# Walter0807/MotionBERT

Hardware: AMD Instinct MI355X
Metric: clips/sec [B,243,17,3] DSTformer fwd+bwd (higher is better)
Workload: dtype bf16; 1 GPU; MotionBERT full DSTformer (dim_feat 512, depth 5, 8 heads, mlp_ratio 2) train step: fwd + bwd + AdamW, 64 clips/GPU x T=243 x J=17, random-init weights, pose loss (mpjpe + 0.5 n_mpjpe + 20 velocity, fused kernel), one-launch flat AdamW; global_batch=64, frames=243, parallelism=dp1

## Files before the change

motionbert_amd/csrc/attention.hip:

```cpp
#include "mbx_common.h"

template <bool SHARED> struct AttnBlock { static constexpr int THREADS = SHARED ? 512 : 256, WAVES = THREADS / 64; };
constexpr int MBX_ATTN_KV_THREADS = 256;
template <bool SHARED> struct AttnBlockKV { static constexpr int THREADS = SHARED ? MBX_ATTN_KV_THREADS : 256, WAVES = THREADS / 64; };

template <typename T> struct AT;
template <> struct AT<bf16_t> { static constexpr int EPC = 8, RB = 8, SZ = 2; };
template <> struct AT<float>  { static constexpr int EPC = 4, RB = 4, SZ = 4; };

template <typename T, int HD> struct BReg;
template <int HD> struct BReg<bf16_t, HD> {
    uint4 v[HD / 16];
    __device__ __forceinline__ void load(const bf16_t* row, int g, bool valid) {
#pragma unroll
        for (int s = 0; s < HD / 16; ++s)
            v[s] = valid ? *reinterpret_cast<const uint4*>(row + 16 * s + 8 * g) : make_uint4(0u, 0u, 0u, 0u);
    }
    static __device__ __forceinline__ float dot(const BReg& a, const BReg& b) {
        float acc = 0.f;
        const uint32_t* x = reinterpret_cast<const uint32_t*>(a.v);
        const uint32_t* y = reinterpret_cast<const uint32_t*>(b.v);
#pragma unroll
        for (int i = 0; i < HD / 4; ++i) {
            acc = fmaf(__uint_as_float(x[i] << 16), __uint_as_float(y[i] << 16), acc);
// ... 499 lines not shown
                tk[c] = *reinterpret_cast<const uint4*>(r3 + C);
                tv[c] = *reinterpret_cast<const uint4*>(r3 + 2 * C);
                td[c] = *reinterpret_cast<const uint4*>(dobase + (size_t)row * ostride + ch * 8);
            }
        }
        if (stats && lane < 3 * HD / 4) {
            const int j = lane / (HD / 4), d = (lane % (HD / 4)) * 4;
            const float4 r = *reinterpret_cast<const float4*>(st_rsum + j * C + P.h * HD + d);
            const float4 b = *reinterpret_cast<const float4*>(st_bias + j * C + P.h * HD + d);
            vec_reg = make_uint4(pack_bf2(r.x, r.y), pack_bf2(r.z, r.w), pack_bf2(-b.x, -b.y), pack_bf2(-b.z, -b.w));
        }
#pragma unroll
        for (int c = 0; c < NPT; ++c) {
            const int idx = lane + c * 64, off = (idx / CHB) * RSTR + (idx % CHB) * 16;
            *reinterpret_cast<uint4*>(qt + off) = tq[c];
            *reinterpret_cast<uint4*>(kt + off) = tk[c];
            *reinterpret_cast<uint4*>(vt + off) = tv[c];
            *reinterpret_cast<uint4*>(dot_ + off) = td[c];
        }
        if (lane < KP) lse_s[lane] = l;
    } else {
        fill_two<T, HD, HD / AT<T>::EPC / 2>(qt, qbase, rstride, kt, qbase + C, rstride, RSTR, P.L, KP, lane, 64);
        fill_two<T, HD, HD / AT<T>::EPC / 2>(vt, qbase + 2 * C, rstride, dot_, dobase, ostride, RSTR, P.L, KP, lane, 64);
        if (stats && lane < 3 * HD / 4) {
            const int j = lane / (HD / 4), d = (lane % (HD / 4)) * 4;
            const float4 r = *reinterpret_cast<const float4*>(st_rsum + j * C + P.h * HD + d);
            const float4 b = *reinterpret_cast<const float4*>(st_bias + j * C + P.h * HD + d);
            vec_reg = make_uint4(pack_bf2(r.x, r.y), pack_bf2(r.z, r.w), pack_bf2(-b.x, -b.y), pack_bf2(-b.z, -b.w));
        }
        if (lane < KP) lse_s[lane] = lane < P.L ? lse[(P.tok0 + (size_t)lane * P.tstep) * H + P.h] : 0.f;
    }
    __syncthreads();
    const bool rvalid = pvalid && i < P.L;
    const size_t tok = P.tok0 + (size_t)min(i, P.L - 1) * P.tstep;

    f32x16_t dq[HD / 32];
    {
        BReg<T, HD> qreg, doreg;
        qreg.load(reinterpret_cast<const T*>(qt + (size_t)i * RSTR), g, true);
        doreg.load(reinterpret_cast<const T*>(dot_ + (size_t)i * RSTR), g, true);
        const float lq = lse_s[i];
        f32x16_t sf, dp;
#pragma unroll
        for (int r = 0; r < 16; ++r) { sf[r] = 0.f; dp[r] = 0.f; }
#pragma unroll
        for (int df = 0; df < HD / 32; ++df)
#pragma unroll
            for (int r = 0; r < 16; ++r) dq[df][r] = 0.f;
        MmaRows<T, HD>::run(kt, RSTR, 0, qreg, lane, sf);
        MmaRows<T, HD>::run(vt, RSTR, 0, doreg, lane, dp);
        float dl = 0.f;
#pragma unroll
        for (int r = 0; r < 16; ++r) {
            const int key = (r & 3) + 8 * (r >> 2) + 4 * g;
            const float pr = (rvalid && key < P.L) ? __expf(sf[r] * scale - lq) : 0.f;
            const float dpr = DROP ? dp[r] * drop_mul(dr, P.dbase, min(i, P.L - 1), min(key, P.L - 1), P.L) : dp[r];
            sf[r] = pr;
            dp[r] = dpr;
            dl = fmaf(pr, dpr, dl);
        }
        const float delta = wave_halves<WaveAdd>(dl);
        if (g == 0) del_s[i] = delta;
#pragma unroll
        for (int r = 0; r < 16; ++r) sf[r] = sf[r] * (dp[r] - delta) * scale;
#pragma unroll
        for (int df = 0; df < HD / 32; ++df) MmaCols<T>::run(kt, RSTR, df * 32, 0, sf, lane, dq[df]);
    }
    {
        BReg<T, HD> kreg, vreg;
        kreg.load(reinterpret_cast<const T*>(kt + (size_t)i * RSTR), g, true);
        vreg.load(reinterpret_cast<const T*>(vt + (size_t)i * RSTR), g, true);
        if (!stats) store_rowfrag<T, HD>(reinterpret_cast<T*>(kt + (size_t)i * RSTR), dq, 1.0f, g);
        f32x16_t sf, dp, dk[HD / 32], dv[HD / 32];
#pragma unroll
        for (int r = 0; r < 16; ++r) { sf[r] = 0.f; dp[r] = 0.f; }
#pragma unroll
        for (int df = 0; df < HD / 32; ++df)
#pragma unroll
            for (int r = 0; r < 16; ++r) { dk[df][r] = 0.f; dv[df][r] = 0.f; }
        MmaRows<T, HD>::run(qt, RSTR, 0, kreg, lane, sf);
        MmaRows<T, HD>::run(dot_, RSTR, 0, vreg, lane, dp);
#pragma unroll
        for (int qd = 0; qd < 4; ++qd) {
            const int q0 = 8 * qd + 4 * g;
            const float4 l4 = *reinterpret_cast<const float4*>(lse_s + q0);
            const float4 d4 = *reinterpret_cast<const float4*>(del_s + q0);
            const float la[4] = {l4.x, l4.y, l4.z, l4.w}, da[4] = {d4.x, d4.y, d4.z, d4.w};
#pragma unroll
            for (int e = 0; e < 4; ++e) {
                const int r = 4 * qd + e;
                const float pr = (rvalid && q0 + e < P.L) ? __expf(sf[r] * scale - la[e]) : 0.f;
                const float km = DROP ? drop_mul(dr, P.dbase, min(q0 + e, P.L - 1), min(i, P.L - 1), P.L) : 1.f;
                dp[r] = pr * (dp[r] * km - da[e]) * scale;
                sf[r] = pr * km;
            }
        }
#pragma unroll
        for (int df = 0; df < HD / 32; ++df) {
            MmaCols<T>::run(dot_, RSTR, df * 32, 0, sf, lane, dv[df]);
            MmaCols<T>::run(qt, RSTR, df * 32, 0, dp, lane, dk[df]);
        }
        if constexpr (sizeof(T) == 2) {
            if (stats) {
                if (lane < 3 * HD / 4) vec[lane] = vec_reg;
                float a1 = 0.f, a2 = 0.f, b1 = 0.f, b2 = 0.f;
                store_rowfrag_dot<HD>(reinterpret_cast<bf16_t*>(qt + (size_t)i * RSTR), dq, g, vec, a1, a2);
                store_rowfrag_dot<HD>(reinterpret_cast<bf16_t*>(kt + (size_t)i * RSTR), dk, g, vec + HD / 4, b1, b2);
                store_rowfrag_dot<HD>(reinterpret_cast<bf16_t*>(vt + (size_t)i * RSTR), dv, g, vec + 2 * (HD / 4), b1, b2);
                a1 = wave_halves<WaveAdd>(a1); a2 = wave_halves<WaveAdd>(a2);
                b1 = wave_halves<WaveAdd>(b1); b2 = wave_halves<WaveAdd>(b2);
                if (rvalid && g == 0) {
                    const size_t Mtot = (size_t)(nprob / H) * P.L;
                    *reinterpret_cast<float2*>(st_part + ((size_t)(2 * P.h) * Mtot + tok) * 2) = make_float2(a1, a2);
                    *reinterpret_cast<float2*>(st_part + ((size_t)(2 * P.h + 1) * Mtot + tok) * 2) = make_float2(b1, b2);
                }
            }
        }
        if (!stats) {
            store_rowfrag<T, HD>(reinterpret_cast<T*>(vt + (size_t)i * RSTR), dk, 1.0f, g);
            store_rowfrag<T, HD>(reinterpret_cast<T*>(qt + (size_t)i * RSTR), dv, 1.0f, g);
        }
    }
    if (pvalid) {
        constexpr int CH = HD * (int)sizeof(T) / 16;
        T* ob = dqkv + P.tok0 * C3 + (size_t)P.h * HD;
        const char* sa = stats ? qt : kt;
        const char* sb = stats ? kt : vt;
        const char* sc = stats ? vt : qt;
        for (int idx = lane; idx < P.L * CH; idx += 64) {
            const int r = idx / CH, ch = idx % CH, off = r * RSTR + ch * 16;
            const uint4 a = *reinterpret_cast<const uint4*>(sa + off);
            const uint4 b = *reinterpret_cast<const uint4*>(sb + off);
            const uint4 c = *reinterpret_cast<const uint4*>(sc + off);
            if (sizeof(T) == 4 && dq_lo) {
                const size_t eo = P.tok0 * C3 + (size_t)P.h * HD + (size_t)r * rstride + ch * 4;
                bf16_t* const hi = reinterpret_cast<bf16_t*>(dqkv);
                const float va[4] = {__uint_as_float(a.x), __uint_as_float(a.y), __uint_as_float(a.z), __uint_as_float(a.w)};
                const float vb[4] = {__uint_as_float(b.x), __uint_as_float(b.y), __uint_as_float(b.z), __uint_as_float(b.w)};
                const float vc[4] = {__uint_as_float(c.x), __uint_as_float(c.y), __uint_as_float(c.z), __uint_as_float(c.w)};
                store4_planes(hi + eo, dq_lo + eo, va);
                store4_planes(hi + eo + C, dq_lo + eo + C, vb);
                store4_planes(hi + eo + 2 * C, dq_lo + eo + 2 * C, vc);
                continue;
            }
            T* dst = ob + (size_t)r * rstride + ch * (16 / (int)sizeof(T));
            *reinterpret_cast<uint4*>(dst) = a;
            *reinterpret_cast<uint4*>(dst + C) = b;
            *reinterpret_cast<uint4*>(dst + 2 * C) = c;
        }
    }
}

__device__ __forceinline__ bf16_t* qt_row(char* tile, int row, int stride) { return reinterpret_cast<bf16_t*>(tile + (size_t)row * stride); }
template <int HD>
__device__ __forceinline__ void mma_rows_ldsb(const char* tile, int stride, int row0, const char* brow, int lane, f32x16_t& acc) {
    const char* p = tile + (size_t)(row0 + (lane & 31)) * stride + (lane >> 5) * 16;
#pragma unroll
    for (int s = 0; s < HD / 16; ++s) {
        const bf16x8_t a = *reinterpret_cast<const bf16x8_t*>(p + s * 32);
        const bf16x8_t b = *reinterpret_cast<const bf16x8_t*>(brow + s * 32);
        acc = __builtin_amdgcn_mfma_f32_32x32x16_bf16(a, b, acc, 0, 0, 0);
    }
}

struct Raw4b {
    static __device__ __forceinline__ void unpack(const uint2& r, float (&v)[4]) {
        v[0] = __uint_as_float(r.x << 16); v[1] = __uint_as_float(r.x & 0xffff0000u);
        v[2] = __uint_as_float(r.y << 16); v[3] = __uint_as_float(r.y & 0xffff0000u);
    }
};
#ifndef MBX_ATTN_DBG
#define MBX_ATTN_DBG 0
#endif
#ifdef MBX_ATTN_TRACE
__device__ long long* g_attn_trace;
#define AT_TS(slot_) do { if (threadIdx.x == 0) ats[slot_] = (long long)wall_clock64(); __builtin_amdgcn_sched_barrier(0); } while (0)
#else
#define AT_TS(slot_) do { } while (0)
#endif
template <int HD, bool STATS>
__global__ __launch_bounds__(1024, 1) void attn_bwd_fused_kernel(const bf16_t* __restrict__ qkv, const bf16_t* __restrict__ o,
                                                                 const bf16_t* __restrict__ d_o, const float* __restrict__ lse,
                                                                 bf16_t* __restrict__ dqkv, int Tn, int J, int H, float scale,
                                                                 int mode, int nprob, int KP, const float* __restrict__ st_bias,
                                                                 const float* __restrict__ st_rsum, float* __restrict__ st_part) {
    typedef bf16_t T;
    constexpr int RSTR = rm_stride<T>(HD), CH = HD / 8;
    extern __shared__ __attribute__((aligned(16))) char smem[];
#ifdef MBX_ATTN_TRACE
    long long ats[8] = {0, 0, 0, 0, 0, 0, 0, 0};
#endif
    AT_TS(0);
    const int tid = threadIdx.x, lane = tid & 63, wave = __builtin_amdgcn_readfirstlane(tid >> 6), g = lane >> 5;
    const int C = H * HD, C3 = 3 * C;
    const Prob P = decode_prob((int)blockIdx.x, mode, Tn, J, H);
    const int TB = KP * RSTR;
    char* qt = smem;
    char* kt = qt + TB;
    char* vt = kt + TB;
    char* dot_ = vt + TB;
    float* lse_s = reinterpret_cast<float*>(dot_ + TB);
    float* del_s = lse_s + KP;
    uint4* vec = reinterpret_cast<uint4*>(del_s + KP);
    const size_t rstride = (size_t)P.tstep * C3, ostride = (size_t)P.tstep * C;
    const T* qbase = qkv + P.tok0 * C3 + (size_t)P.h * HD;
    const T* dobase = d_o + P.tok0 * C + (size_t)P.h * HD;
    const T* obase = o + P.tok0 * C + (size_t)P.h * HD;
    if (STATS) fill_stat_vec<HD>(vec, st_rsum, st_bias, C, P.h, tid, 1024);

    for (int i0 = tid; i0 < KP * CH; i0 += 2048) {
        uint4 v[2][4], vo[2];
        float sl[2] = {0.f, 0.f};
#pragma unroll
        for (int u = 0; u < 2; ++u) {
            const int idx = i0 + u * 1024, row = idx / CH, ch = idx % CH;
#pragma unroll
            for (int t = 0; t < 4; ++t) v[u][t] = make_uint4(0u, 0u, 0u, 0u);
            vo[u] = make_uint4(0u, 0u, 0u, 0u);
            if (idx < KP * CH && row < P.L && !(MBX_ATTN_DBG & 4)) {
                const T* r3 = qbase + (size_t)row * rstride + ch * 8;
                v[u][0] = *reinterpret_cast<const uint4*>(r3);
                v[u][1] = *reinterpret_cast<const uint4*>(r3 + C);
                v[u][2] = *reinterpret_cast<const uint4*>(r3 + 2 * C);
                v[u][3] = *reinterpret_cast<const uint4*>(dobase + (size_t)row * ostride + ch * 8);
                vo[u] = *reinterpret_cast<const uint4*>(obase + (size_t)row * ostride + ch * 8);
                if (ch == 0) sl[u] = lse[(P.tok0 + (size_t)row * P.tstep) * H + P.h];
            }
        }
#pragma unroll
        for (int u = 0; u < 2; ++u) {
            const int idx = i0 + u * 1024, row = idx / CH, ch = idx % CH;
            if (idx < KP * CH) {
                const int off = row * RSTR + ch * 16;
                *reinterpret_cast<uint4*>(qt + off) = v[u][0];
                *reinterpret_cast<uint4*>(kt + off) = v[u][1];
                *reinterpret_cast<uint4*>(vt + off) = v[u][2];
                *reinterpret_cast<uint4*>(dot_ + off) = v[u][3];
            }
        }
        AT_TS(1);
#pragma unroll
        for (int u = 0; u < 2; ++u) {
            const int idx = i0 + u * 1024, row = idx / CH, ch = idx % CH;
            float x[4], y[4], dl = 0.f;
            Raw4b::unpack(make_uint2(v[u][3].x, v[u][3].y), x); Raw4b::unpack(make_uint2(vo[u].x, vo[u].y), y);
            dl = fmaf(x[0], y[0], fmaf(x[1], y[1], fmaf(x[2], y[2], fmaf(x[3], y[3], dl))));
            Raw4b::unpack(make_uint2(v[u][3].z, v[u][3].w), x); Raw4b::unpack(make_uint2(vo[u].z, vo[u].w), y);
            dl = fmaf(x[0], y[0], fmaf(x[1], y[1], fmaf(x[2], y[2], fmaf(x[3], y[3], dl))));
            dl += dpp_mov<0xB1>(dl, dl);
            dl += dpp_mov<0x4E>(dl, dl);
            if (CH == 8) dl += dpp_mov<0x141>(dl, dl);
            if (ch == 0 && idx < KP * CH) {
                lse_s[row] = sl[u] * 1.44269504088896341f;
                del_s[row] = dl;
            }
        }
    }
    __syncthreads();
    AT_TS(2);

    const int nfr = (P.L + 31) / 32;
    const float c2 = scale * 1.44269504088896341f;
    f32x16_t acc[2 * (HD / 32)];
#pragma unroll
    for (int a = 0; a < 2 * (HD / 32); ++a)
#pragma unroll
        for (int r = 0; r < 16; ++r) acc[a][r] = 0.f;
    const bool qrole = wave >= 8;
    const int blk = wave & 7, row = blk * 32 + (lane & 31);
    if (blk < nfr && !(MBX_ATTN_DBG & 1)) {
        if (qrole) {
            BReg<T, HD> qreg, doreg;
            qreg.load(reinterpret_cast<const T*>(qt + (size_t)row * RSTR), g, true);
            doreg.load(reinterpret_cast<const T*>(dot_ + (size_t)row * RSTR), g, true);
            const float delta = del_s[row], lq2 = lse_s[row];
            for (int f = 0; f < nfr; ++f) {
                f32x16_t s, dp;
#pragma unroll
                for (int r = 0; r < 16; ++r) { s[r] = 0.f; dp[r] = 0.f; }
                MmaRows<T, HD>::run(kt, RSTR, 32 * f, qreg, lane, s);
                MmaRows<T, HD>::run(vt, RSTR, 32 * f, doreg, lane, dp);
#pragma unroll
                for (int r = 0; r < 16; ++r) {
                    const float p = __builtin_amdgcn_exp2f(fmaf(s[r], c2, -lq2));
                    s[r] = p * (dp[r] - delta);
                }
#pragma unroll
                for (int df = 0; df < HD / 32; ++df) MmaCols<T>::run(kt, RSTR, df * 32, f, s, lane, acc[df]);
            }
        } else {
            int boff = row * RSTR + g * 16;
            for (int f = 0; f < nfr; ++f) {
                asm volatile("" : "+v"(boff));
                f32x16_t s, dp;
#pragma unroll
                for (int r = 0; r < 16; ++r) { s[r] = 0.f; dp[r] = 0.f; }
                mma_rows_ldsb<HD>(qt, RSTR, 32 * f, kt + boff, lane, s);
                mma_rows_ldsb<HD>(dot_, RSTR, 32 * f, vt + boff, lane, dp);
#pragma unroll
                for (int qd = 0; qd < 4; ++qd) {
                    const int q0 = 32 * f + 8 * qd + 4 * g;
                    const float4 l4 = *reinterpret_cast<const float4*>(lse_s + q0);
                    const float4 d4 = *reinterpret_cast<const float4*>(del_s + q0);
                    const float la[4] = {l4.x, l4.y, l4.z, l4.w}, da[4] = {d4.x, d4.y, d4.z, d4.w};
#pragma unroll
                    for (int e = 0; e < 4; ++e) {
                        const int r = 4 * qd + e;
                        const float p = __builtin_amdgcn_exp2f(fmaf(s[r], c2, -la[e]));
                        dp[r] = p * (dp[r] - da[e]);
                        s[r] = p;
                    }
                }
#pragma unroll
                for (int df = 0; df < HD / 32; ++df) {
                    MmaCols<T>::run(dot_, RSTR, df * 32, f, s, lane, acc[HD / 32 + df]);
                    MmaCols<T>::run(qt, RSTR, df * 32, f, dp, lane, acc[df]);
                }
            }
        }
#pragma unroll
        for (int a = 0; a < HD / 32; ++a)
#pragma unroll
            for (int r = 0; r < 16; ++r) acc[a][r] *= scale;
    }
    AT_TS(3);
#ifdef MBX_ATTN_TRACE
    if (g_attn_trace != nullptr && (threadIdx.x & 63) == 0) g_attn_trace[(size_t)gridDim.x * 9 + (size_t)blockIdx.x * 16 + (threadIdx.x >> 6)] = (long long)wall_clock64();
#endif
    __syncthreads();
    AT_TS(4);
    int tid2 = threadIdx.x;
    asm volatile("" : "+v"(tid2));
    const int g2 = (tid2 >> 5) & 1, row2 = blk * 32 + (tid2 & 31);
    const bool qrole2 = wave >= 8;
    if (blk < nfr) {
        if (STATS) {
            float p1 = 0.f, p2 = 0.f;
            if (qrole2) {
                store_rowfrag_dot<HD>(qt_row(qt, row2, RSTR), reinterpret_cast<const f32x16_t (&)[HD / 32]>(acc[0]), g2, vec, p1, p2);
            } else {
                store_rowfrag_dot<HD>(qt_row(kt, row2, RSTR), reinterpret_cast<const f32x16_t (&)[HD / 32]>(acc[0]), g2, vec + HD / 4, p1, p2);
                store_rowfrag_dot<HD>(qt_row(vt, row2, RSTR), reinterpret_cast<const f32x16_t (&)[HD / 32]>(acc[HD / 32]), g2, vec + 2 * (HD / 4), p1, p2);
            }
            p1 = wave_halves<WaveAdd>(p1);
            p2 = wave_halves<WaveAdd>(p2);
            if (g2 == 0 && row2 < P.L) {
                const size_t Mtot = (size_t)(nprob / H) * P.L;
                *reinterpret_cast<float2*>(st_part + ((size_t)(2 * P.h + (qrole2 ? 0 : 1)) * Mtot + P.tok0 + (size_t)row2 * P.tstep) * 2) = make_float2(p1, p2);
            }
        } else if (qrole2) {
            store_rowfrag<T, HD>(reinterpret_cast<T*>(qt + (size_t)row2 * RSTR), reinterpret_cast<const f32x16_t (&)[HD / 32]>(acc[0]), 1.0f, g2);
        } else {
            store_rowfrag<T, HD>(reinterpret_cast<T*>(kt + (size_t)row2 * RSTR), reinterpret_cast<const f32x16_t (&)[HD / 32]>(acc[0]), 1.0f, g2);
            store_rowfrag<T, HD>(reinterpret_cast<T*>(vt + (size_t)row2 * RSTR), reinterpret_cast<const f32x16_t (&)[HD / 32]>(acc[HD / 32]), 1.0f, g2);
        }
    }
    __syncthreads();
    AT_TS(5);
    T* obase3 = dqkv + P.tok0 * C3 + (size_t)P.h * HD;
    for (int i0 = tid2; i0 < KP * CH; i0 += 2048) {
        uint4 v[2][3];
#pragma unroll
        for (int u = 0; u < 2; ++u) {
            const int idx = min(i0 + u * 1024, KP * CH - 1), off = (idx / CH) * RSTR + (idx % CH) * 16;
            v[u][0] = *reinterpret_cast<const uint4*>(qt + off);
            v[u][1] = *reinterpret_cast<const uint4*>(kt + off);
            v[u][2] = *reinterpret_cast<const uint4*>(vt + off);
        }
#pragma unroll
        for (int u = 0; u < 2; ++u) {
            const int idx = i0 + u * 1024, r = idx / CH, ch = idx % CH;
            if (idx < KP * CH && r < P.L && !(MBX_ATTN_DBG & 2)) {
                T* r3 = obase3 + (size_t)r * rstride + ch * 8;
                *reinterpret_cast<uint4*>(r3) = v[u][0];
                *reinterpret_cast<uint4*>(r3 + C) = v[u][1];
                *reinterpret_cast<uint4*>(r3 + 2 * C) = v[u][2];
            }
        }
    }
#ifdef MBX_ATTN_TRACE
    AT_TS(6);
    asm volatile("s_waitcnt vmcnt(0)" ::: "memory");
    AT_TS(7);
    if (g_attn_trace != nullptr && threadIdx.x == 0) {
        long long* const tr = g_attn_trace + (size_t)blockIdx.x * 9;
#pragma unroll
        for (int k = 0; k < 8; ++k) tr[k] = ats[k];
        tr[8] = (long long)__builtin_amdgcn_s_getreg(63492) | ((long long)__builtin_amdgcn_s_getreg(63508) << 32);
    }
#endif
}

static int check_attn_args(const char* who, int B, int T, int J, int H, int hd, int mode, int dtype) {
    MBX_CHECK_ARG(B > 0 && T > 0 && J > 0 && H > 0, "%s: bad shape", who);
    MBX_CHECK_ARG(hd == 32 || hd == 64, "%s: head dim %d unsupported (32 or 64)", who, hd);
    MBX_CHECK_ARG(mode == MBX_ATTN_SPATIAL || mode == MBX_ATTN_TEMPORAL, "%s: unknown mode %d", who, mode);
    MBX_CHECK_ARG(dtype == MBX_BF16 || dtype == MBX_F32, "%s: unknown dtype %d", who, dtype);
    const int L = mode == MBX_ATTN_SPATIAL ? J : T;
    MBX_CHECK_ARG(L <= 256, "%s: sequence length %d > 256 unsupported", who, L);
    return 0;
}

template <typename K>
static int set_lds(K kernel, size_t bytes, const char* who) {
    if (bytes > 160 * 1024) return mbx_set_error("%s: needs %zu bytes of LDS (> 160 KiB)", who, bytes);
    return bytes > 64 * 1024 ? mbx_set_dyn_lds(reinterpret_cast<const void*>(kernel), bytes, who) : 0;
}

static int make_drop(const char* who, float p, uint64_t seed, MbxDrop& dr) {
    MBX_CHECK_ARG(p >= 0.f && p < 1.f, "%s: dropout rate %g outside [0, 1)", who, (double)p);
    dr.seed_lo = (uint32_t)seed;
    dr.seed_hi = (uint32_t)(seed >> 32);
    dr.thresh = p > 0.f ? (uint32_t)fminf(p * 4294967296.0f, 4294967295.0f) : 0u;
    dr.scale = p > 0.f ? 1.0f / (1.0f - p) : 1.0f;
    return 0;
}

template <typename T, int HD, bool SHARED, bool DROP>
static int launch_fwd(const void* qkv, void* o, float* lse, int Tn, int J, int H, float scale, int mode, int nprob, int KP, hipStream_t s,
                      const MbxDrop& dr) {
    constexpr bool IS_BF = sizeof(T) == 2;
    const size_t per = (size_t)2 * KP * rm_stride<T>(HD);
    const size_t shm = SHARED ? per : 4 * per;
    auto kern = attn_fwd_kernel<T, HD, SHARED, DROP>;
    if (set_lds(kern, shm, "attn_fwd")) return 1;
    const int grid = SHARED ? nprob : (nprob + 3) / 4;
    hipLaunchKernelGGL(kern, dim3(grid), dim3(AttnBlock<SHARED>::THREADS), shm, s, (const T*)qkv, (T*)o, lse, Tn, J, H, scale, mode, nprob, KP, dr);
    MBX_LAUNCH_CHECK("attn_fwd");
    return 0;
}

static int attn_fwd_impl(const void* qkv, void* o, float* lse, int B, int T, int J, int H, int hd, float scale, int mode,
                         int dtype, void* stream, const MbxDrop& dr) {
    MBX_CHECK_ARG(qkv && o && lse, "attn_fwd: null pointer");
    MBX_CHECK_ARG(scale > 0.f, "attn_fwd: scale must be positive (the running max is taken over the raw scores), got %g", (double)scale);
    if (check_attn_args("attn_fwd", B, T, J, H, hd, mode, dtype)) return 1;
    const int L = mode == MBX_ATTN_SPATIAL ? J : T;
    const int nprob = mode == MBX_ATTN_SPATIAL ? B * T * H : B * J * H;
    const int KP = ((L + 31) / 32) * 32;
    const bool shared = KP > 32;
    hipStream_t s = (hipStream_t)stream;
#define MBX_FWD2(TT, HDV, DR)                                                                        \
    (shared ? launch_fwd<TT, HDV, true, DR>(qkv, o, lse, T, J, H, scale, mode, nprob, KP, s, dr)       \
            : launch_fwd<TT, HDV, false, DR>(qkv, o, lse, T, J, H, scale, mode, nprob, KP, s, dr))
#define MBX_FWD(TT, HDV) (dr.thresh ? MBX_FWD2(TT, HDV, true) : MBX_FWD2(TT, HDV, false))
    if (dtype == MBX_BF16) return hd == 64 ? MBX_FWD(bf16_t, 64) : MBX_FWD(bf16_t, 32);
    return hd == 64 ? MBX_FWD(float, 64) : MBX_FWD(float, 32);
#undef MBX_FWD
#undef MBX_FWD2
}
extern "C" int mbx_attn_fwd(const void* qkv, void* o, float* lse, int B, int T, int J, int H, int hd, float scale, int mode,
                            int dtype, void* stream) {
    MbxDrop dr;
    make_drop("attn_fwd", 0.f, 0, dr);
    return attn_fwd_impl(qkv, o, lse, B, T, J, H, hd, scale, mode, dtype, stream, dr);
}
extern "C" int mbx_attn_fwd_drop(const void* qkv, void* o, float* lse, int B, int T, int J, int H, int hd, float scale, int mode,
                                 int dtype, float p, uint64_t seed, void* stream) {
    MbxDrop dr;
    if (make_drop("attn_fwd_drop", p, seed, dr)) return 1;
    return attn_fwd_impl(qkv, o, lse, B, T, J, H, hd, scale, mode, dtype, stream, dr);
}

template <typename T, int HD, bool SHARED, bool DROP>
static int launch_bwd(const void* qkv, const void* o, const void* d_o, const float* lse, void* dqkv, int Tn, int J, int H,
                      float scale, int mode, int nprob, int KP, hipStream_t s, const MbxDrop& dr, void* dq_lo) {
    constexpr bool IS_BF = sizeof(T) == 2;
    const int RSTR = rm_stride<T>(HD);
    const size_t per_dq = (size_t)2 * KP * RSTR;
    const size_t per_dkv = (size_t)2 * KP * RSTR + 2 * KP * 4;
    const int grid = SHARED ? nprob : (nprob + 3) / 4;
    auto k1 = attn_bwd_dq_kernel<T, HD, SHARED, DROP>;
    auto k2 = attn_bwd_dkv_kernel<T, HD, SHARED, DROP>;
    const size_t shm1 = SHARED ? per_dq : 4 * per_dq, shm2 = SHARED ? per_dkv : 4 * per_dkv;
    if (set_lds(k1, shm1, "attn_bwd_dq") || set_lds(k2, shm2, "attn_bwd_dkv")) return 1;
    hipLaunchKernelGGL(k1, dim3(grid), dim3(AttnBlock<SHARED>::THREADS), shm1, s, (const T*)qkv, (const T*)o, (const T*)d_o, lse, (T*)dqkv, Tn, J, H, scale, mode, nprob, KP, dr, (bf16_t*)dq_lo);
    MBX_LAUNCH_CHECK("attn_bwd_dq");
    hipLaunchKernelGGL(k2, dim3(grid), dim3(AttnBlockKV<SHARED>::THREADS), shm2, s, (const T*)qkv, (const T*)o, (const T*)d_o, lse, (T*)dqkv, Tn, J, H, scale, mode, nprob, KP, dr, (bf16_t*)dq_lo);
    MBX_LAUNCH_CHECK("attn_bwd_dkv");
    return 0;
}

#ifdef MBX_ATTN_TRACE
#define MBX_ATTN_TRACE_SET(s_) do { static long long* const tb = [] { const char* e = getenv("MBX_TRACE_BUF"); return e ? (long long*)strtoull(e, nullptr, 0) : (long long*)nullptr; }(); \
                                    (void)hipMemcpyToSymbolAsync(HIP_SYMBOL(g_attn_trace), &tb, sizeof(tb), 0, hipMemcpyHostToDevice, (s_)); } while (0)
#else
#define MBX_ATTN_TRACE_SET(s_) do { } while (0)
#endif
static int attn_bwd_impl(const void* qkv, const void* o, const void* d_o, const float* lse, void* dqkv, int B, int T, int J,
                         int H, int hd, float scale, int mode, int dtype, void* stream, const float* st_bias, const float* st_rsum,
                         float* st_part, const MbxDrop& dr, void* dq_lo = nullptr) {
    MBX_CHECK_ARG(qkv && o && d_o && lse && dqkv, "attn_bwd: null pointer");
    MBX_CHECK_ARG(!dq_lo || dtype == MBX_F32, "attn_bwd: operand planes are an output form of the fp32 kernels");
    MBX_CHECK_ARG(!(st_part && dr.thresh), "attn_bwd: the row dots of the folded LayerNorm backward and dropout do not combine");
    if (check_attn_args("attn_bwd", B, T, J, H, hd, mode, dtype)) return 1;
    const int L = mode == MBX_ATTN_SPATIAL ? J : T;
    const int nprob = mode == MBX_ATTN_SPATIAL ? B * T * H : B * J * H;
    const int KP = ((L + 31) / 32) * 32;
    const bool shared = KP > 32;
    hipStream_t s = (hipStream_t)stream;
    if (shared && dtype == MBX_BF16 && !dr.thresh) {
        const size_t shm = (size_t)4 * KP * rm_stride<bf16_t>(hd) + 2 * KP * 4 + 3 * hd * 4;
        if (shm <= 160 * 1024) {
#define MBX_BWD_FUSED(HDV)                                                                                            \
    do {                                                                                                              \
        auto k = st_part ? attn_bwd_fused_kernel<HDV, true> : attn_bwd_fused_kernel<HDV, false>;                     \
        if (set_lds(k, shm, "attn_bwd_fused")) return 1;                                                              \
        MBX_ATTN_TRACE_SET(s);                                                                                        \
        hipLaunchKernelGGL(k, dim3(nprob), dim3(1024), shm, s, (const bf16_t*)qkv, (const bf16_t*)o, (const bf16_t*)d_o, lse, \
                           (bf16_t*)dqkv, T, J, H, scale, mode, nprob, KP, st_bias, st_rsum, st_part);                \
        MBX_LAUNCH_CHECK("attn_bwd_fused");                                                                           \
        return 0;                                                                                                     \
    } while (0)
            if (hd == 64) MBX_BWD_FUSED(64); else MBX_BWD_FUSED(32);
#undef MBX_BWD_FUSED
        }
    }
    if (!shared) {
#define MBX_BWD_SMALL2(TT, HDV, DR)                                                                                   \
    do {                                                                                                              \
        const size_t shm = (size_t)4 * (4 * 32 * rm_stride<TT>(HDV) + 2 * 32 * 4);                                    \
        auto k = attn_bwd_small_kernel<TT, HDV, DR>;                                                                  \
        if (set_lds(k, shm, "attn_bwd_small")) return 1;                                                              \
        hipLaunchKernelGGL(k, dim3((nprob + 3) / 4), dim3(256), shm, s, (const TT*)qkv, (const TT*)o, (const TT*)d_o, lse, \
                           (TT*)dqkv, T, J, H, scale, mode, nprob, st_bias, st_rsum, st_part, dr, (bf16_t*)dq_lo);   \
        MBX_LAUNCH_CHECK("attn_bwd_small");                                                                           \
        return 0;                                                                                                     \
    } while (0)
#define MBX_BWD_SMALL(TT, HDV) do { if (dr.thresh) MBX_BWD_SMALL2(TT, HDV, true); else MBX_BWD_SMALL2(TT, HDV, false); } while (0)
        if (dtype == MBX_BF16) { if (hd == 64) MBX_BWD_SMALL(bf16_t, 64); else MBX_BWD_SMALL(bf16_t, 32); }
        else { if (hd == 64) MBX_BWD_SMALL(float, 64); else MBX_BWD_SMALL(float, 32); }
#undef MBX_BWD_SMALL
#undef MBX_BWD_SMALL2
    }
    MBX_CHECK_ARG(!st_part, "attn_bwd_stats: this shape runs the two-kernel backward, which has no row-dot output");
#define MBX_BWD2(TT, HDV, DR)                                                                                         \
    (shared ? launch_bwd<TT, HDV, true, DR>(qkv, o, d_o, lse, dqkv, T, J, H, scale, mode, nprob, KP, s, dr, dq_lo)    \
            : launch_bwd<TT, HDV, false, DR>(qkv, o, d_o, lse, dqkv, T, J, H, scale, mode, nprob, KP, s, dr, dq_lo))
#define MBX_BWD(TT, HDV) (dr.thresh ? MBX_BWD2(TT, HDV, true) : MBX_BWD2(TT, HDV, false))
    if (dtype == MBX_BF16) return hd == 64 ? MBX_BWD(bf16_t, 64) : MBX_BWD(bf16_t, 32);
    return hd == 64 ? MBX_BWD(float, 64) : MBX_BWD(float, 32);
#undef MBX_BWD
#undef MBX_BWD2
}

extern "C" int mbx_attn_bwd(const void* qkv, const void* o, const void* d_o, const float* lse, void* dqkv, int B, int T, int J,
                            int H, int hd, float scale, int mode, int dtype, void* stream) {
    MbxDrop dr;
    make_drop("attn_bwd", 0.f, 0, dr);
    return attn_bwd_impl(qkv, o, d_o, lse, dqkv, B, T, J, H, hd, scale, mode, dtype, stream, nullptr, nullptr, nullptr, dr);
}
extern "C" int mbx_attn_bwd_planes(const void* qkv, const void* o, const void* d_o, const float* lse, void* dqkv_hi, void* dqkv_lo, int B,
                                   int T, int J, int H, int hd, float scale, int mode, float p, uint64_t seed, void* stream) {
    MBX_CHECK_ARG(dqkv_lo, "attn_bwd_planes: null pointer");
    MbxDrop dr;
    if (make_drop("attn_bwd_planes", p, seed, dr)) return 1;
    return attn_bwd_impl(qkv, o, d_o, lse, dqkv_hi, B, T, J, H, hd, scale, mode, MBX_F32, stream, nullptr, nullptr, nullptr, dr, dqkv_lo);
}
extern "C" int mbx_attn_bwd_drop(const void* qkv, const void* o, const void* d_o, const float* lse, void* dqkv, int B, int T, int J,
                                 int H, int hd, float scale, int mode, int dtype, float p, uint64_t seed, void* stream) {
    MbxDrop dr;
    if (make_drop("attn_bwd_drop", p, seed, dr)) return 1;
    return attn_bwd_impl(qkv, o, d_o, lse, dqkv, B, T, J, H, hd, scale, mode, dtype, stream, nullptr, nullptr, nullptr, dr);
}
extern "C" int mbx_attn_bwd_stats(const void* qkv, const void* o, const void* d_o, const float* lse, void* dqkv, const float* bias_f,
                                  const float* rsum, float* part, int B, int T, int J, int H, int hd, float scale, int mode,
                                  void* stream) {
    MBX_CHECK_ARG(bias_f && rsum && part, "attn_bwd_stats: null pointer");
    MBX_CHECK_ARG((reinterpret_cast<uintptr_t>(part) & 7) == 0, "attn_bwd_stats: part must be 8-byte aligned");
    MbxDrop dr;
    make_drop("attn_bwd_stats", 0.f, 0, dr);
    return attn_bwd_impl(qkv, o, d_o, lse, dqkv, B, T, J, H, hd, scale, mode, MBX_BF16, stream, bias_f, rsum, part, dr);
}
```

Before: 585.7 clips/s.

## Restructure temporal attention backward into flash-style chunked pipeline with dedicated dQ waves

```diff
diff --git a/motionbert_amd/csrc/attention.hip b/motionbert_amd/csrc/attention.hip
--- a/motionbert_amd/csrc/attention.hip
+++ b/motionbert_amd/csrc/attention.hip
@@ -675,16 +675,6 @@
 }
 
 __device__ __forceinline__ bf16_t* qt_row(char* tile, int row, int stride) { return reinterpret_cast<bf16_t*>(tile + (size_t)row * stride); }
-template <int HD>
-__device__ __forceinline__ void mma_rows_ldsb(const char* tile, int stride, int row0, const char* brow, int lane, f32x16_t& acc) {
-    const char* p = tile + (size_t)(row0 + (lane & 31)) * stride + (lane >> 5) * 16;
-#pragma unroll
-    for (int s = 0; s < HD / 16; ++s) {
-        const bf16x8_t a = *reinterpret_cast<const bf16x8_t*>(p + s * 32);
-        const bf16x8_t b = *reinterpret_cast<const bf16x8_t*>(brow + s * 32);
-        acc = __builtin_amdgcn_mfma_f32_32x32x16_bf16(a, b, acc, 0, 0, 0);
-    }
-}
 
 struct Raw4b {
     static __device__ __forceinline__ void unpack(const uint2& r, float (&v)[4]) {
@@ -692,6 +682,14 @@
         v[2] = __uint_as_float(r.y << 16); v[3] = __uint_as_float(r.y & 0xffff0000u);
     }
 };
+__device__ __forceinline__ bf16x8_t tr_frag(const char* tile, int stride, int row0, int col0, int lane) {
+    const int g = lane >> 5, r16 = lane & 15;
+    const char* a0 = tile + (size_t)(row0 + 4 * g + (r16 >> 2)) * stride + (col0 + 16 * ((lane >> 4) & 1) + 4 * (r16 & 3)) * 2;
+    union { v4s_t h[2]; bf16x8_t v; } a;
+    a.h[0] = __builtin_amdgcn_ds_read_tr16_b64_v4i16((lds_v4s_t*)a0);
+    a.h[1] = __builtin_amdgcn_ds_read_tr16_b64_v4i16((lds_v4s_t*)(a0 + (size_t)8 * stride));
+    return a.v;
+}
 #ifndef MBX_ATTN_DBG
 #define MBX_ATTN_DBG 0
 #endif
@@ -701,14 +699,32 @@
 #else
 #define AT_TS(slot_) do { } while (0)
 #endif
+template <int HD> struct AttnFA {
+    static constexpr int NKW = 8;
+    static constexpr int NQW = 4;
+    static constexpr int THREADS = 64 * (NKW + NQW);
+    static constexpr int NDF = HD / 32;
+    static constexpr int NPH = NQW / NDF;
+    static constexpr int NSL = NPH + 1;
+    static constexpr int QC = 32;
+    static constexpr int RSTR = rm_stride<bf16_t>(HD);
+    static constexpr int DSTR = QC * 2 + 8;
+    static constexpr int SSTR = 32 * 2 + 16;
+    static constexpr int QTB = QC * RSTR;
+    static constexpr size_t lds(int KP) {
+        return (size_t)2 * KP * RSTR + 4 * QTB + 4 * QC * 4 + (size_t)NSL * KP * DSTR + NQW * QC * SSTR + NQW * QC * 8 + 12 * HD;
+    }
+};
 template <int HD, bool STATS>
-__global__ __launch_bounds__(1024, 1) void attn_bwd_fused_kernel(const bf16_t* __restrict__ qkv, const bf16_t* __restrict__ o,
-                                                                 const bf16_t* __restrict__ d_o, const float* __restrict__ lse,
-                                                                 bf16_t* __restrict__ dqkv, int Tn, int J, int H, float scale,
-                                                                 int mode, int nprob, int KP, const float* __restrict__ st_bias,
-                                                                 const float* __restrict__ st_rsum, float* __restrict__ st_part) {
+__global__ __launch_bounds__(AttnFA<HD>::THREADS, 1) void attn_bwd_fa_kernel(const bf16_t* __restrict__ qkv, const bf16_t* __restrict__ o,
+                                                                              const bf16_t* __restrict__ d_o, const float* __restrict__ lse,
+                                                                              bf16_t* __restrict__ dqkv, int Tn, int J, int H, float scale,
+                                                                              int mode, int nprob, int KP, const float* __restrict__ st_bias,
+                                                                              const float* __restrict__ st_rsum, float* __restrict__ st_part) {
     typedef bf16_t T;
-    constexpr int RSTR = rm_stride<T>(HD), CH = HD / 8;
+    typedef AttnFA<HD> F;
+    constexpr int RSTR = F::RSTR, DSTR = F::DSTR, SSTR = F::SSTR, QTB = F::QTB, QC = F::QC, CH = HD / 8;
+    constexpr int NPH = F::NPH, NSL = F::NSL, NDF = F::NDF;
     extern __shared__ __attribute__((aligned(16))) char smem[];
 #ifdef MBX_ATTN_TRACE
     long long ats[8] = {0, 0, 0, 0, 0, 0, 0, 0};
@@ -717,114 +733,101 @@
     const int tid = threadIdx.x, lane = tid & 63, wave = __builtin_amdgcn_readfirstlane(tid >> 6), g = lane >> 5;
     const int C = H * HD, C3 = 3 * C;
     const Prob P = decode_prob((int)blockIdx.x, mode, Tn, J, H);
-    const int TB = KP * RSTR;
-    char* qt = smem;
-    char* kt = qt + TB;
-    char* vt = kt + TB;
-    char* dot_ = vt + TB;
-    float* lse_s = reinterpret_cast<float*>(dot_ + TB);
-    float* del_s = lse_s + KP;
-    uint4* vec = reinterpret_cast<uint4*>(del_s + KP);
+    char* kt = smem;
+    char* vt = kt + KP * RSTR;
+    char* qs = vt + KP * RSTR;
+    char* dos = qs + 2 * QTB;
+    float* lses = reinterpret_cast<float*>(dos + 2 * QTB);
+    float* dels = lses + 2 * QC;
+    char* dss = reinterpret_cast<char*>(dels + 2 * QC);
+    char* stg = dss + (size_t)NSL * KP * DSTR;
+    float2* parts = reinterpret_cast<float2*>(stg + F::NQW * QC * SSTR);
+    uint4* vec = reinterpret_cast<uint4*>(parts + F::NQW * QC);
     const size_t rstride = (size_t)P.tstep * C3, ostride = (size_t)P.tstep * C;
     const T* qbase = qkv + P.tok0 * C3 + (size_t)P.h * HD;
     const T* dobase = d_o + P.tok0 * C + (size_t)P.h * HD;
     const T* obase = o + P.tok0 * C + (size_t)P.h * HD;
-    if (STATS) fill_stat_vec<HD>(vec, st_rsum, st_bias, C, P.h, tid, 1024);
-
-    for (int i0 = tid; i0 < KP * CH; i0 += 2048) {
-        uint4 v[2][4], vo[2];
-        float sl[2] = {0.f, 0.f};
-#pragma unroll
-        for (int u = 0; u < 2; ++u) {
-            const int idx = i0 + u * 1024, row = idx / CH, ch = idx % CH;
-#pragma unroll
-            for (int t = 0; t < 4; ++t) v[u][t] = make_uint4(0u, 0u, 0u, 0u);
-            vo[u] = make_uint4(0u, 0u, 0u, 0u);
-            if (idx < KP * CH && row < P.L && !(MBX_ATTN_DBG & 4)) {
-                const T* r3 = qbase + (size_t)row * rstride + ch * 8;
-                v[u][0] = *reinterpret_cast<const uint4*>(r3);
-                v[u][1] = *reinterpret_cast<const uint4*>(r3 + C);
-                v[u][2] = *reinterpret_cast<const uint4*>(r3 + 2 * C);
-                v[u][3] = *reinterpret_cast<const uint4*>(dobase + (size_t)row * ostride + ch * 8);
-                vo[u] = *reinterpret_cast<const uint4*>(obase + (size_t)row * ostride + ch * 8);
-                if (ch == 0) sl[u] = lse[(P.tok0 + (size_t)row * P.tstep) * H + P.h];
-            }
-        }
-#pragma unroll
-        for (int u = 0; u < 2; ++u) {
-            const int idx = i0 + u * 1024, row = idx / CH, ch = idx % CH;
-            if (idx < KP * CH) {
-                const int off = row * RSTR + ch * 16;
-                *reinterpret_cast<uint4*>(qt + off) = v[u][0];
-                *reinterpret_cast<uint4*>(kt + off) = v[u][1];
-                *reinterpret_cast<uint4*>(vt + off) = v[u][2];
-                *reinterpret_cast<uint4*>(dot_ + off) = v[u][3];
-            }
-        }
-        AT_TS(1);
-#pragma unroll
-        for (int u = 0; u < 2; ++u) {
-            const int idx = i0 + u * 1024, row = idx / CH, ch = idx % CH;
-            float x[4], y[4], dl = 0.f;
-            Raw4b::unpack(make_uint2(v[u][3].x, v[u][3].y), x); Raw4b::unpack(make_uint2(vo[u].x, vo[u].y), y);
-            dl = fmaf(x[0], y[0], fmaf(x[1], y[1], fmaf(x[2], y[2], fmaf(x[3], y[3], dl))));
-            Raw4b::unpack(make_uint2(v[u][3].z, v[u][3].w), x); Raw4b::unpack(make_uint2(vo[u].z, vo[u].w), y);
-            dl = fmaf(x[0], y[0], fmaf(x[1], y[1], fmaf(x[2], y[2], fmaf(x[3], y[3], dl))));
-            dl += dpp_mov<0xB1>(dl, dl);
-            dl += dpp_mov<0x4E>(dl, dl);
-            if (CH == 8) dl += dpp_mov<0x141>(dl, dl);
-            if (ch == 0 && idx < KP * CH) {
-                lse_s[row] = sl[u] * 1.44269504088896341f;
-                del_s[row] = dl;
-            }
-        }
-    }
+    const size_t Mtot = (size_t)(nprob / H) * P.L;
+    if (STATS) fill_stat_vec<HD>(vec, st_rsum, st_bias, C, P.h, tid, F::THREADS);
+    const int nfr = (P.L + 31) / 32;
+    const float c2 = scale * 1.44269504088896341f;
+
+    const bool qwave = wave >= F::NKW;
+    const int lt = tid - 64 * F::NKW;
+    const bool loader = qwave && lt < QC * CH;
+    const int lrow = lt / CH, lch = lt % CH;
+    uint4 cq, cd, co;
+    float cl = 0.f;
+    auto load_chunk = [&](int c) {
+        cq = cd = co = make_uint4(0u, 0u, 0u, 0u);
+        cl = 0.f;
+        const int row = c * QC + lrow;
+        if (row < P.L && !(MBX_ATTN_DBG & 4)) {
+            cq = *reinterpret_cast<const uint4*>(qbase + (size_t)row * rstride + lch * 8);
+            cd = *reinterpret_cast<const uint4*>(dobase + (size_t)row * ostride + lch * 8);
+            co = *reinterpret_cast<const uint4*>(obase + (size_t)row * ostride + lch * 8);
+            if (lch == 0) cl = lse[(P.tok0 + (size_t)row * P.tstep) * H + P.h];
+        }
+    };
+    auto store_chunk = [&](int c) {
+        const int sl = c & 1, off = lrow * RSTR + lch * 16;
+        *reinterpret_cast<uint4*>(qs + sl * QTB + off) = cq;
+        *reinterpret_cast<uint4*>(dos + sl * QTB + off) = cd;
+        float x[4], y[4], dl = 0.f;
+        Raw4b::unpack(make_uint2(cd.x, cd.y), x); Raw4b::unpack(make_uint2(co.x, co.y), y);
+        dl = fmaf(x[0], y[0], fmaf(x[1], y[1], fmaf(x[2], y[2], fmaf(x[3], y[3], dl))));
+        Raw4b::unpack(make_uint2(cd.z, cd.w), x); Raw4b::unpack(make_uint2(co.z, co.w), y);
+        dl = fmaf(x[0], y[0], fmaf(x[1], y[1], fmaf(x[2], y[2], fmaf(x[3], y[3], dl))));
+        dl += dpp_mov<0xB1>(dl, dl);
+        dl += dpp_mov<0x4E>(dl, dl);
+        if (CH == 8) dl += dpp_mov<0x141>(dl, dl);
+        if (lch == 0) {
+            lses[sl * QC + lrow] = cl * 1.44269504088896341f;
+            dels[sl * QC + lrow] = dl;
+        }
+    };
+
+    if (loader) load_chunk(0);
+    {
+        constexpr int NPT = (256 * CH + F::THREADS - 1) / F::THREADS;
+        uint4 v0[NPT], v1[NPT];
+        fill_two<T, HD, NPT>(kt, qbase + C, rstride, vt, qbase + 2 * C, rstride, RSTR, (MBX_ATTN_DBG & 4) ? 0 : P.L, KP, tid, F::THREADS, v0, v1);
+    }
+    AT_TS(1);
+    if (loader) store_chunk(0);
     __syncthreads();
     AT_TS(2);
 
-    const int nfr = (P.L + 31) / 32;
-    const float c2 = scale * 1.44269504088896341f;
-    f32x16_t acc[2 * (HD / 32)];
-#pragma unroll
-    for (int a = 0; a < 2 * (HD / 32); ++a)
-#pragma unroll
-        for (int r = 0; r < 16; ++r) acc[a][r] = 0.f;
-    const bool qrole = wave >= 8;
-    const int blk = wave & 7, row = blk * 32 + (lane & 31);
-    if (blk < nfr && !(MBX_ATTN_DBG & 1)) {
-        if (qrole) {
-            BReg<T, HD> qreg, doreg;
-            qreg.load(reinterpret_cast<const T*>(qt + (size_t)row * RSTR), g, true);
-            doreg.load(reinterpret_cast<const T*>(dot_ + (size_t)row * RSTR), g, true);
-            const float delta = del_s[row], lq2 = lse_s[row];
-            for (int f = 0; f < nfr; ++f) {
+    if (!qwave) {
+        const int key = wave * 32 + (lane & 31);
+        const bool kwave = wave < nfr;
+        BReg<T, HD> kreg, vreg;
+        f32x16_t dk[NDF], dv[NDF];
+#pragma unroll
+        for (int df = 0; df < NDF; ++df)
+#pragma unroll
+            for (int r = 0; r < 16; ++r) { dk[df][r] = 0.f; dv[df][r] = 0.f; }
+        if (kwave) {
+            kreg.load(reinterpret_cast<const T*>(kt + (size_t)key * RSTR), g, true);
+            vreg.load(reinterpret_cast<const T*>(vt + (size_t)key * RSTR), g, true);
+        }
+        for (int c = 0; c < nfr + NPH; ++c) {
+            if (kwave && c < nfr && !(MBX_ATTN_DBG & 1)) {
+                const char* qc = qs + (c & 1) * QTB;
+                const char* dc = dos + (c & 1) * QTB;
+                const float* lc = lses + (c & 1) * QC;
+                const float* ec = dels + (c & 1) * QC;
                 f32x16_t s, dp;
 #pragma unroll
                 for (int r = 0; r < 16; ++r) { s[r] = 0.f; dp[r] = 0.f; }
-                MmaRows<T, HD>::run(kt, RSTR, 32 * f, qreg, lane, s);
-                MmaRows<T, HD>::run(vt, RSTR, 32 * f, doreg, lane, dp);
-#pragma unroll
-                for (int r = 0; r < 16; ++r) {
-                    const float p = __builtin_amdgcn_exp2f(fmaf(s[r], c2, -lq2));
-                    s[r] = p * (dp[r] - delta);
-                }
-#pragma unroll
-                for (int df = 0; df < HD / 32; ++df) MmaCols<T>::run(kt, RSTR, df * 32, f, s, lane, acc[df]);
-            }
-        } else {
-            int boff = row * RSTR + g * 16;
-            for (int f = 0; f < nfr; ++f) {
-                asm volatile("" : "+v"(boff));
-                f32x16_t s, dp;
-#pragma unroll
-                for (int r = 0; r < 16; ++r) { s[r] = 0.f; dp[r] = 0.f; }
-                mma_rows_ldsb<HD>(qt, RSTR, 32 * f, kt + boff, lane, s);
-                mma_rows_ldsb<HD>(dot_, RSTR, 32 * f, vt + boff, lane, dp);
+                MmaRows<T, HD>::run(qc, RSTR, 0, kreg, lane, s);
+                MmaRows<T, HD>::run(dc, RSTR, 0, vreg, lane, dp);
+                char* dsw = dss + (size_t)(c % NSL) * KP * DSTR + (size_t)key * DSTR + 8 * g;
 #pragma unroll
                 for (int qd = 0; qd < 4; ++qd) {
-                    const int q0 = 32 * f + 8 * qd + 4 * g;
-                    const float4 l4 = *reinterpret_cast<const float4*>(lse_s + q0);
-                    const float4 d4 = *reinterpret_cast<const float4*>(del_s + q0);
+                    const int q0 = 8 * qd + 4 * g;
+                    const float4 l4 = *reinterpret_cast<const float4*>(lc + q0);
+                    const float4 d4 = *reinterpret_cast<const float4*>(ec + q0);
                     const float la[4] = {l4.x, l4.y, l4.z, l4.w}, da[4] = {d4.x, d4.y, d4.z, d4.w};
 #pragma unroll
                     for (int e = 0; e < 4; ++e) {
@@ -833,72 +836,132 @@
                         dp[r] = p * (dp[r] - da[e]);
                         s[r] = p;
                     }
+                    *reinterpret_cast<uint2*>(dsw + 16 * qd) = make_uint2(pack_bf2(dp[4 * qd], dp[4 * qd + 1]), pack_bf2(dp[4 * qd + 2], dp[4 * qd + 3]));
                 }
 #pragma unroll
-                for (int df = 0; df < HD / 32; ++df) {
-                    MmaCols<T>::run(dot_, RSTR, df * 32, f, s, lane, acc[HD / 32 + df]);
-                    MmaCols<T>::run(qt, RSTR, df * 32, f, dp, lane, acc[df]);
+                for (int df = 0; df < NDF; ++df) {
+                    MmaCols<T>::run(dc, RSTR, df * 32, 0, s, lane, dv[df]);
+                    MmaCols<T>::run(qc, RSTR, df * 32, 0, dp, lane, dk[df]);
                 }
             }
-        }
-#pragma unroll
-        for (int a = 0; a < HD / 32; ++a)
-#pragma unroll
-            for (int r = 0; r < 16; ++r) acc[a][r] *= scale;
-    }
-    AT_TS(3);
 #ifdef MBX_ATTN_TRACE
-    if (g_attn_trace != nullptr && (threadIdx.x & 63) == 0) g_attn_trace[(size_t)gridDim.x * 9 + (size_t)blockIdx.x * 16 + (threadIdx.x >> 6)] = (long long)wall_clock64();
+            if (c == nfr - 1 && g_attn_trace != nullptr && (threadIdx.x & 63) == 0)
+                g_attn_trace[(size_t)gridDim.x * 9 + (size_t)blockIdx.x * 16 + (threadIdx.x >> 6)] = (long long)wall_clock64();
 #endif
-    __syncthreads();
+            __syncthreads();
+        }
+        AT_TS(3);
+        if (kwave) {
+#pragma unroll
+            for (int df = 0; df < NDF; ++df)
+#pragma unroll
+                for (int r = 0; r < 16; ++r) dk[df][r] *= scale;
+            if (STATS) {
+                float p1 = 0.f, p2 = 0.f;
+                store_rowfrag_dot<HD>(qt_row(kt, key, RSTR), dk, g, vec + HD / 4, p1, p2);
+                store_rowfrag_dot<HD>(qt_row(vt, key, RSTR), dv, g, vec + 2 * (HD / 4), p1, p2);
+                p1 = wave_halves<WaveAdd>(p1);
+                p2 = wave_halves<WaveAdd>(p2);
+                if (g == 0 && key < P.L)
+                    *reinterpret_cast<float2*>(st_part + ((size_t)(2 * P.h + 1) * Mtot + P.tok0 + (size_t)key * P.tstep) * 2) = make_float2(p1, p2);
+            } else {
+                store_rowfrag<T, HD>(reinterpret_cast<T*>(kt + (size_t)key * RSTR), dk, 1.0f, g);
+                store_rowfrag<T, HD>(reinterpret_cast<T*>(vt + (size_t)key * RSTR), dv, 1.0f, g);
+            }
+        }
+    } else {
+        const int qw = wave - F::NKW;
+        const int qdf = qw % NDF, qph = qw / NDF;
+        char* stg_w = stg + qw * QC * SSTR;
+        f32x16_t dq;
+#pragma unroll
+        for (int r = 0; r < 16; ++r) dq[r] = 0.f;
+        int pend = -1;
+        auto flush_parts = [&]() {
+            if (qdf == 0 && lane < QC) {
+                const float2 a = parts[(qph * 2) * QC + lane], b = parts[(qph * 2 + 1) * QC + lane];
+                const int row = pend * QC + lane;
+                if (row < P.L)
+                    *reinterpret_cast<float2*>(st_part + ((size_t)(2 * P.h) * Mtot + P.tok0 + (size_t)row * P.tstep) * 2) = make_float2(a.x + b.x, a.y + b.y);
+            }
+            pend = -1;
+        };
+        for (int c = 0; c < nfr + NPH; ++c) {
+            const bool pre = loader && c + 1 < nfr;
+            if (pre) load_chunk(c + 1);
+            if (STATS && NDF == 2 && pend >= 0) flush_parts();
+            const int d = c - 1 - qph;
+            if (d >= 0 && c - 1 - d % NPH < nfr) {
+                const int j = c - 1 - d % NPH, s = d % NPH;
+                const char* dsr = dss + (size_t)(j % NSL) * KP * DSTR;
+                if (!(MBX_ATTN_DBG & 1)) {
+                    for (int f = s * nfr / NPH; f < (s + 1) * nfr / NPH; ++f) {
+#pragma unroll
+                        for (int t = 0; t < 2; ++t) {
+                            const bf16x8_t b = tr_frag(dsr, DSTR, 32 * f + 16 * t, 0, lane);
+                            const bf16x8_t a = tr_frag(kt, RSTR, 32 * f + 16 * t, 32 * qdf, lane);
+                            dq = __builtin_amdgcn_mfma_f32_32x32x16_bf16(a, b, dq, 0, 0, 0);
+                        }
+                    }
+                }
+                if (s == NPH - 1) {
+                    const int q = lane & 31;
+#pragma unroll
+                    for (int qd = 0; qd < 4; ++qd)
+                        *reinterpret_cast<uint2*>(stg_w + q * SSTR + (8 * qd + 4 * g) * 2) =
+                            make_uint2(pack_bf2(dq[4 * qd] * scale, dq[4 * qd + 1] * scale), pack_bf2(dq[4 * qd + 2] * scale, dq[4 * qd + 3] * scale));
+#pragma unroll
+                    for (int r = 0; r < 16; ++r) dq[r] = 0.f;
+#pragma unroll
+                    for (int u = 0; u < 2; ++u) {
+                        const int idx = lane + 64 * u, r = idx >> 2, ch = idx & 3, row = j * QC + r;
+                        const uint4 v = *reinterpret_cast<const uint4*>(stg_w + r * SSTR + ch * 16);
+                        const size_t eo = (size_t)row * rstride + qdf * 32 + ch * 8;
+                        if (row < P.L && !(MBX_ATTN_DBG & 2)) *reinterpret_cast<uint4*>(dqkv + P.tok0 * C3 + (size_t)P.h * HD + eo) = v;
+                        if (STATS) {
+                            uint4 qo = make_uint4(0u, 0u, 0u, 0u);
+                            if (row < P.L) qo = *reinterpret_cast<const uint4*>(qbase + eo);
+                            const uint4 va = vec[(qdf * 32 + ch * 8) / 4], vb = vec[(qdf * 32 + ch * 8) / 4 + 1];
+                            float p1 = dot2_bf16(v.x, va.x, dot2_bf16(v.y, va.y, 0.f));
+                            p1 = dot2_bf16(v.z, vb.x, dot2_bf16(v.w, vb.y, p1));
+                            float p2 = dot2_bf16(v.x, qo.x, dot2_bf16(v.y, qo.y, dot2_bf16(v.x, va.z, dot2_bf16(v.y, va.w, 0.f))));
+                            p2 = dot2_bf16(v.z, qo.z, dot2_bf16(v.w, qo.w, dot2_bf16(v.z, vb.z, dot2_bf16(v.w, vb.w, p2))));
+                            p1 += dpp_mov<0xB1>(p1, p1); p1 += dpp_mov<0x4E>(p1, p1);
+                            p2 += dpp_mov<0xB1>(p2, p2); p2 += dpp_mov<0x4E>(p2, p2);
+                            if (ch == 0) {
+                                if (NDF == 1) {
+                                    if (row < P.L)
+                                        *reinterpret_cast<float2*>(st_part + ((size_t)(2 * P.h) * Mtot + P.tok0 + (size_t)row * P.tstep) * 2) = make_float2(p1, p2);
+                                } else {
+                                    parts[(qph * 2 + qdf) * QC + r] = make_float2(p1, p2);
+                                }
+                            }
+                        }
+                    }
+                    if (STATS && NDF == 2) pend = j;
+                }
+            }
+            if (pre) store_chunk(c + 1);
+#ifdef MBX_ATTN_TRACE
+            if (c == nfr + NPH - 1 && g_attn_trace != nullptr && (threadIdx.x & 63) == 0)
+                g_attn_trace[(size_t)gridDim.x * 9 + (size_t)blockIdx.x * 16 + (threadIdx.x >> 6)] = (long long)wall_clock64();
+#endif
+            __syncthreads();
+        }
+        if (STATS && NDF == 2 && pend >= 0) flush_parts();
+    }
     AT_TS(4);
-    int tid2 = threadIdx.x;
-    asm volatile("" : "+v"(tid2));
-    const int g2 = (tid2 >> 5) & 1, row2 = blk * 32 + (tid2 & 31);
-    const bool qrole2 = wave >= 8;
-    if (blk < nfr) {
-        if (STATS) {
-            float p1 = 0.f, p2 = 0.f;
-            if (qrole2) {
-                store_rowfrag_dot<HD>(qt_row(qt, row2, RSTR), reinterpret_cast<const f32x16_t (&)[HD / 32]>(acc[0]), g2, vec, p1, p2);
-            } else {
-                store_rowfrag_dot<HD>(qt_row(kt, row2, RSTR), reinterpret_cast<const f32x16_t (&)[HD / 32]>(acc[0]), g2, vec + HD / 4, p1, p2);
-                store_rowfrag_dot<HD>(qt_row(vt, row2, RSTR), reinterpret_cast<const f32x16_t (&)[HD / 32]>(acc[HD / 32]), g2, vec + 2 * (HD / 4), p1, p2);
-            }
-            p1 = wave_halves<WaveAdd>(p1);
-            p2 = wave_halves<WaveAdd>(p2);
-            if (g2 == 0 && row2 < P.L) {
-                const size_t Mtot = (size_t)(nprob / H) * P.L;
-                *reinterpret_cast<float2*>(st_part + ((size_t)(2 * P.h + (qrole2 ? 0 : 1)) * Mtot + P.tok0 + (size_t)row2 * P.tstep) * 2) = make_float2(p1, p2);
-            }
-        } else if (qrole2) {
-            store_rowfrag<T, HD>(reinterpret_cast<T*>(qt + (size_t)row2 * RSTR), reinterpret_cast<const f32x16_t (&)[HD / 32]>(acc[0]), 1.0f, g2);
-        } else {
-            store_rowfrag<T, HD>(reinterpret_cast<T*>(kt + (size_t)row2 * RSTR), reinterpret_cast<const f32x16_t (&)[HD / 32]>(acc[0]), 1.0f, g2);
-            store_rowfrag<T, HD>(reinterpret_cast<T*>(vt + (size_t)row2 * RSTR), reinterpret_cast<const f32x16_t (&)[HD / 32]>(acc[HD / 32]), 1.0f, g2);
-        }
-    }
     __syncthreads();
     AT_TS(5);
     T* obase3 = dqkv + P.tok0 * C3 + (size_t)P.h * HD;
-    for (int i0 = tid2; i0 < KP * CH; i0 += 2048) {
-        uint4 v[2][3];
-#pragma unroll
-        for (int u = 0; u < 2; ++u) {
-            const int idx = min(i0 + u * 1024, KP * CH - 1), off = (idx / CH) * RSTR + (idx % CH) * 16;
-            v[u][0] = *reinterpret_cast<const uint4*>(qt + off);
-            v[u][1] = *reinterpret_cast<const uint4*>(kt + off);
-            v[u][2] = *reinterpret_cast<const uint4*>(vt + off);
-        }
-#pragma unroll
-        for (int u = 0; u < 2; ++u) {
-            const int idx = i0 + u * 1024, r = idx / CH, ch = idx % CH;
-            if (idx < KP * CH && r < P.L && !(MBX_ATTN_DBG & 2)) {
-                T* r3 = obase3 + (size_t)r * rstride + ch * 8;
-                *reinterpret_cast<uint4*>(r3) = v[u][0];
-                *reinterpret_cast<uint4*>(r3 + C) = v[u][1];
-                *reinterpret_cast<uint4*>(r3 + 2 * C) = v[u][2];
-            }
+    for (int idx = tid; idx < P.L * CH; idx += F::THREADS) {
+        const int r = idx / CH, ch = idx % CH, off = r * RSTR + ch * 16;
+        const uint4 a = *reinterpret_cast<const uint4*>(kt + off);
+        const uint4 b = *reinterpret_cast<const uint4*>(vt + off);
+        if (!(MBX_ATTN_DBG & 2)) {
+            T* r3 = obase3 + (size_t)r * rstride + ch * 8;
+            *reinterpret_cast<uint4*>(r3 + C) = a;
+            *reinterpret_cast<uint4*>(r3 + 2 * C) = b;
         }
     }
 #ifdef MBX_ATTN_TRACE
@@ -1023,21 +1086,19 @@
     const bool shared = KP > 32;
     hipStream_t s = (hipStream_t)stream;
     if (shared && dtype == MBX_BF16 && !dr.thresh) {
-        const size_t shm = (size_t)4 * KP * rm_stride<bf16_t>(hd) + 2 * KP * 4 + 3 * hd * 4;
-        if (shm <= 160 * 1024) {
-#define MBX_BWD_FUSED(HDV)                                                                                            \
+#define MBX_BWD_FA(HDV)                                                                                               \
     do {                                                                                                              \
-        auto k = st_part ? attn_bwd_fused_kernel<HDV, true> : attn_bwd_fused_kernel<HDV, false>;                     \
-        if (set_lds(k, shm, "attn_bwd_fused")) return 1;                                                              \
+        const size_t shm = AttnFA<HDV>::lds(KP);                                                                      \
+        auto k = st_part ? attn_bwd_fa_kernel<HDV, true> : attn_bwd_fa_kernel<HDV, false>;                           \
+        if (set_lds(k, shm, "attn_bwd_fa")) return 1;                                                                 \
         MBX_ATTN_TRACE_SET(s);                                                                                        \
-        hipLaunchKernelGGL(k, dim3(nprob), dim3(1024), shm, s, (const bf16_t*)qkv, (const bf16_t*)o, (const bf16_t*)d_o, lse, \
-                           (bf16_t*)dqkv, T, J, H, scale, mode, nprob, KP, st_bias, st_rsum, st_part);                \
-        MBX_LAUNCH_CHECK("attn_bwd_fused");                                                                           \
+        hipLaunchKernelGGL(k, dim3(nprob), dim3(AttnFA<HDV>::THREADS), shm, s, (const bf16_t*)qkv, (const bf16_t*)o,  \
+                           (const bf16_t*)d_o, lse, (bf16_t*)dqkv, T, J, H, scale, mode, nprob, KP, st_bias, st_rsum, st_part); \
+        MBX_LAUNCH_CHECK("attn_bwd_fa");                                                                              \
         return 0;                                                                                                     \
     } while (0)
-            if (hd == 64) MBX_BWD_FUSED(64); else MBX_BWD_FUSED(32);
-#undef MBX_BWD_FUSED
-        }
+        if (hd == 64) MBX_BWD_FA(64); else MBX_BWD_FA(32);
+#undef MBX_BWD_FA
     }
     if (!shared) {
 #define MBX_BWD_SMALL2(TT, HDV, DR)                                                                                   \
```

After: 590.3 clips/s (median of 6 runs). About the same (+0.8%).
